# nkkk98/MyGPURaytracer

Hardware: AMD Instinct MI355X
Metric: Mrays/s (higher is better)
Workload: dtype f32; 1 GPU; cornellObj.txt 1920x1080 depth 8, AA on, material sort on, 1 spp/step (BASELINE configs[3] / C4); arith=0, clock_warmup_steps=1152, rccl_ranks=1, parallelism=1 GPU

## Files before the change

include/mi355x_pathtracer.h:

```cpp
#ifndef MI355X_PATHTRACER_H
#define MI355X_PATHTRACER_H

#include <stddef.h>
#include <stdint.h>

#ifdef __cplusplus
extern "C" {
#endif

#define PTX_ABI_VERSION 5
int ptx_abi_version(void);
size_t ptx_sizeof_options(void);
size_t ptx_sizeof_stats(void);

#define PTX_OK 0
#define PTX_ERR_INVALID 1
#define PTX_ERR_IO 2
#define PTX_ERR_HIP 3
#define PTX_ERR_NODEVICE 4
#define PTX_ERR_UNSUPPORTED 5

enum { PTX_SPHERE = 0, PTX_CUBE = 1, PTX_TRIANGLE = 2, PTX_OBJ = 3 };

typedef struct ptx_material {
// ... 217 lines not shown
                          int spp);

int ptx_kat_geom_test(ptx_tracer *t, int geom, int n, const float *rays6, float *out10);
int ptx_kat_obj_tri_test(ptx_tracer *t, int geom, int n, const float *rays6, float *out8);
int ptx_kat_jittered_hemisphere(ptx_tracer *t, int n, const float *normals3, const int32_t *seeds3, int max_iter, float *out3);
int ptx_kat_compute_intersections(ptx_tracer *t, int n, const void *paths44, void *isects32);
int ptx_kat_tile_intersect(ptx_tracer *t, int n, const void *paths44, void *isects32, int split);
int ptx_kat_shade(ptx_tracer *t, int iter, int n, const int32_t *idx, const void *isects32, void *paths44);
int ptx_kat_generate(ptx_tracer *t, int iter, void *paths44);
int ptx_kat_libm(ptx_tracer *t, int n, const float *x, float *sin_out, float *cos_out,
                 const double *pw_in, double *pow5_out, const float *powf_xy, float *powf_out);
int ptx_kat_fast_exact(ptx_tracer *t, int64_t mismatches[3]);
int ptx_debug_tile_geoms(const ptx_camera *camera, int ngeoms, const float *boxes6, int depth_of_field, int tile_rows, int tile_rank,
                         int tile_world, uint32_t *masks_out, int max_tiles);
int ptx_debug_record_masks(int nmaterials, const ptx_material *materials, int ngeoms, const int32_t *geom_type, const int32_t *geom_material,
                           int sort_by_material, uint64_t masks[2]);
int ptx_debug_cull_boxes(int n, const float *boxes6, float *centre_half8);
int ptx_debug_light_bits(int nmaterials, const ptx_material *materials, int ngeoms, const int32_t *geom_material, uint32_t *bits_out);
int ptx_debug_bounce_occupancy(ptx_tracer *t, int lds_bytes);
int ptx_debug_aux_nonzero(ptx_tracer *t, int64_t out3[3]);
int ptx_debug_set_capture(ptx_tracer *t, int bounce);
int ptx_debug_bvh_check(const float *faces15, int nfaces, const float *rays6, int nrays, int32_t *face_loop, float *t_loop,
                        int32_t *face_bvh, float *t_bvh, int64_t *stats4);
int ptx_debug_bvh_visits(int64_t out8[8]);
int ptx_debug_read_stamps(ptx_tracer *t, unsigned long long out48[48]);
int ptx_debug_read_stream(ptx_tracer *t, int *n_out, int32_t *pixel_index, int32_t *stream_idx,
                          int32_t *material, float *fields14, int cap);

#ifdef __cplusplus
}
#endif
#endif
```

mygpuraytracer_amd/csrc/pt_device.h:

```cpp
#pragma once
#include <hip/hip_runtime.h>
#include <stdint.h>

#define PT_DEV __device__ __forceinline__
#define PT_HD __host__ __device__ __forceinline__

#ifndef PT_ARITH
#define PT_ARITH 0
#endif

namespace ptd {

struct vec3 { float x, y, z; };

PT_HD vec3 V3(float x, float y, float z) { vec3 r; r.x = x; r.y = y; r.z = z; return r; }
PT_HD vec3 add(vec3 a, vec3 b) { return V3(a.x + b.x, a.y + b.y, a.z + b.z); }
PT_HD vec3 sub(vec3 a, vec3 b) { return V3(a.x - b.x, a.y - b.y, a.z - b.z); }
PT_HD vec3 mul(vec3 a, vec3 b) { return V3(a.x * b.x, a.y * b.y, a.z * b.z); }
PT_HD vec3 scale(vec3 a, float s) { return V3(a.x * s, a.y * s, a.z * s); }
PT_HD vec3 neg(vec3 a) { return V3(-a.x, -a.y, -a.z); }
PT_HD float dot(vec3 a, vec3 b) { return a.x * b.x + a.y * b.y + a.z * b.z; }
PT_HD vec3 cross(vec3 x, vec3 y) { return V3(x.y * y.z - y.y * x.z, x.z * y.x - y.z * x.x, x.x * y.y - y.x * x.y); }
#ifndef PT_FAST_EXACT
#define PT_FAST_EXACT 1
// ... 249 lines not shown
    const float *__restrict__ tri9;
    const uint8_t *__restrict__ texels;
    int32_t ngeoms, nmats;
    int32_t tri_lds;
    int32_t ntri;
    int32_t ntri_lds;
    const float *__restrict__ gtab;
    const float *__restrict__ aabb;
    uint32_t cube_bits, sphere_bits, mesh_bits;
    uint32_t light_bits;
    const BvhQuad *__restrict__ bvh_nodes;
    const float *__restrict__ bvh_tris;
    const int32_t *__restrict__ bvh_root;
    const int32_t *__restrict__ bvh_depth;
    int32_t bvh_stack;
    const BvhWide4 *__restrict__ bvh_wide;
    const int32_t *__restrict__ bvh_wroot;
    const int32_t *__restrict__ bvh_wneed;
    const float *__restrict__ fnorm;
    const float *__restrict__ cnorm;
    uint32_t bump_bits;
    int32_t mesh_chunks;
    int32_t cull;
    const float *__restrict__ ldsblob;
};

__host__ __device__ constexpr int sceneTableWords(int ntri_lds, int nmats, int ngeoms) { return (ntri_lds * 27 + nmats * 11 + ngeoms * 58 + 3) & ~3; }
PT_DEV int sceneLdsWords(const DScene &sc) { return sceneTableWords(sc.ntri_lds, sc.nmats, sc.ngeoms); }
constexpr int GTAB_WORDS = 40;

extern __shared__ __attribute__((aligned(16))) int32_t pt_lds[];

__device__ __forceinline__ void stageSceneToLds(const DScene &sc, int tid, int nthreads) {
    float *l = reinterpret_cast<float *>(pt_lds);
    if (sc.ldsblob) {
        const int n = sc.ntri_lds * 27 + sc.nmats * 11 + sc.ngeoms * 58;
        for (int k = tid; k < n; k += 4 * nthreads) {
            const int k1 = k + nthreads, k2 = k1 + nthreads, k3 = k2 + nthreads;
            const float a0 = sc.ldsblob[k], a1 = k1 < n ? sc.ldsblob[k1] : 0.f, a2 = k2 < n ? sc.ldsblob[k2] : 0.f, a3 = k3 < n ? sc.ldsblob[k3] : 0.f;
            l[k] = a0;
            if (k1 < n) l[k1] = a1;
            if (k2 < n) l[k2] = a2;
            if (k3 < n) l[k3] = a3;
        }
        return;
    }
    const int n9 = sc.ntri_lds * 9, n15 = sc.ntri_lds * 15, nm = sc.nmats * 11;
    for (int k = tid; k < n9; k += nthreads) l[k] = sc.tri9[k];
    for (int k = tid; k < n15; k += nthreads) l[n9 + k] = sc.faces[k];
    const float *m = reinterpret_cast<const float *>(sc.mats);
    for (int k = tid; k < nm; k += nthreads) l[n9 + n15 + k] = m[k];
    const int ng = sc.ngeoms * GTAB_WORDS;
// ... 162 lines not shown
    const float tiny = 1e-20f;
    const float ddx = __builtin_fabsf(d.x) < tiny ? __builtin_copysignf(tiny, d.x) : d.x;
    const float ddy = __builtin_fabsf(d.y) < tiny ? __builtin_copysignf(tiny, d.y) : d.y;
    const float ddz = __builtin_fabsf(d.z) < tiny ? __builtin_copysignf(tiny, d.z) : d.z;
    RaySlab r;
    r.ix = 1.0f / ddx; r.iy = 1.0f / ddy; r.iz = 1.0f / ddz;
    r.ox = o.x * r.ix; r.oy = o.y * r.iy; r.oz = o.z * r.iz;
    r.sx = slack * __builtin_fabsf(r.ix); r.sy = slack * __builtin_fabsf(r.iy); r.sz = slack * __builtin_fabsf(r.iz);
    return r;
}
PT_HD bool slabEntry(const BvhQuad &A, const BvhQuad &B, const RaySlab &r, float tmin, float &tn) {
    const float x0 = __builtin_fmaf(A.x, r.ix, -r.ox), x1 = __builtin_fmaf(B.x, r.ix, -r.ox);
    const float y0 = __builtin_fmaf(A.y, r.iy, -r.oy), y1 = __builtin_fmaf(B.y, r.iy, -r.oy);
    const float z0 = __builtin_fmaf(A.z, r.iz, -r.oz), z1 = __builtin_fmaf(B.z, r.iz, -r.oz);
    tn = __builtin_fmaxf(__builtin_fmaxf(__builtin_fminf(x0, x1) - r.sx, __builtin_fminf(y0, y1) - r.sy), __builtin_fminf(z0, z1) - r.sz);
    const float tf = __builtin_fminf(__builtin_fminf(__builtin_fmaxf(x0, x1) + r.sx, __builtin_fmaxf(y0, y1) + r.sy), __builtin_fmaxf(z0, z1) + r.sz);
    return !((tf < tn) || (tf < 0.0f) || (tn > tmin * 1.0001f));
}
PT_HD float bvhSlack(const BvhQuad &A, const BvhQuad &B, vec3 o) {
    const vec3 c = V3(0.5f * (A.x + B.x), 0.5f * (A.y + B.y), 0.5f * (A.z + B.z));
    const vec3 h = V3(0.5f * (B.x - A.x), 0.5f * (B.y - A.y), 0.5f * (B.z - A.z));
    const float s = 1.220703125e-4f * (length(sub(o, c)) + 4.0f * length(h));
    return s == s ? s : 3.0e38f;
}

PT_HD float bvhNearest(const BvhQuad *__restrict__ nodes, const float *__restrict__ tris, int root, vec3 o, vec3 d,
                       int &face, float &b0o, float &b1o, int *visited = nullptr) {
    const RaySlab rs = makeRaySlab(o, d, bvhSlack(nodes[2 * root], nodes[2 * root + 1], o));
    float tmin = 3.402823466e+38f;
    face = -1; b0o = 0.f; b1o = 0.f;
    int n = root;
    while (n >= 0) {
        const BvhQuad A = nodes[2 * n], B = nodes[2 * n + 1];
        float tn_;
        const bool skip = !slabEntry(A, B, rs, tmin, tn_);
        if (visited) ++*visited;
        if (skip) { n = A.w; continue; }
        const int count = (int)((uint32_t)B.w >> 28), first = B.w & 0x0fffffff;
        if (count == 0) { n = n + 1; continue; }
        for (int k = 0; k < count; k++) {
            const float *T = tris + (size_t)(first + k) * BVH_TRI;
            const vec3 v0 = V3(T[0], T[1], T[2]), p1 = V3(T[3], T[4], T[5]), p2 = V3(T[6], T[7], T[8]);
            const vec3 e1 = sub(p1, v0), e2 = sub(p2, v0);
            float b0, b1;
            if (rayTriangle(o, d, v0, e1, e2, b0, b1)) {
                const float w = 1 - b0 - b1;
// ... 869 lines not shown
```

mygpuraytracer_amd/csrc/pt_engine.hip:

```cpp
#include <hip/hip_runtime.h>
#include <stdint.h>
#include <stdio.h>
#include <string.h>
#include <string>
#include <vector>
#include <algorithm>
#include <cmath>

#include "../../include/mi355x_pathtracer.h"
#include "pt_kernels.h"
#include "pt_scene.h"
#include "pt_denoise.h"

namespace {

thread_local std::string g_last_error;
int set_error(int code, const std::string &msg) { g_last_error = msg; return code; }

#define HIPCHECK(expr)                                                                                   \
    do {                                                                                                 \
        hipError_t e_ = (expr);                                                                          \
        if (e_ != hipSuccess)                                                                            \
            return set_error(PTX_ERR_HIP, std::string(#expr) + ": " + hipGetErrorString(e_));            \
    } while (0)
// ... 266 lines not shown
    DevBuf<float> d_var;
    bool var_done = false;
    DevBuf<unsigned long long> d_stamps;
    DevBuf<float> d_part;
    DevBuf<int32_t> d_cache_totals;
    DevBuf<int32_t> d_emit_count, d_emit_pix; DevBuf<float> d_emit_rgb;
    DevBuf<int64_t> d_stats;
    uint32_t fence_slots = 0;
    int maxBounces = 0;
    bool cache_valid = false;
    int64_t iterations = 0;
    double loop_ms_total = 0.0;
    bool ktiming = false;
    std::vector<hipEvent_t> kev;
    std::vector<int> kev_kind;
    size_t kev_used = 0;
    int capture_bounce = -1;
    DevBuf<int32_t> d_cap;
    DevBuf<float> d_cap_f;
    bool cap_filled = false;
    DScene scene() const {
        DScene s; s.geoms = d_geoms; s.mats = d_mats; s.faces = d_faces; s.tri9 = d_tri9; s.texels = d_texels; s.ngeoms = ngeoms; s.nmats = nmats;
        s.gtab = d_gtab; s.aabb = d_aabb; s.cull = 0; s.cube_bits = cube_bits; s.sphere_bits = sphere_bits; s.mesh_bits = mesh_bits; s.light_bits = light_bits;
        s.bvh_nodes = d_bvh_nodes; s.bvh_tris = d_bvh_tris; s.bvh_root = d_bvh_root; s.bvh_depth = d_bvh_depth; s.bvh_wide = d_bvh_wide; s.bvh_wroot = d_bvh_wroot; s.bvh_wneed = d_bvh_wneed; s.bvh_stack = 0; s.ntri_lds = 0; s.mesh_chunks = mesh_chunks;
        s.fnorm = d_fnorm; s.cnorm = d_cnorm; s.bump_bits = bump_bits;
        s.tri_lds = 0; s.ntri = ntri;
        s.ldsblob = nullptr;
        return s;
    }
    bool cache_active() const { return opt.cache_first_bounce && !opt.antialiasing && !opt.depth_of_field; }
    const KernelSet *ks = static_cast<const KernelSet *>(ptx_arith_kernels_0());
    const LastKernelSet *ksl = static_cast<const LastKernelSet *>(ptx_arith_last_0());
};

namespace {

void carve(PathSoA &s, float *f, int32_t *i, size_t stride) {
    s.q = f; s.i = i; s.stride = (uint32_t)stride;
}

PathSoA soa_shift(PathSoA s, size_t off) {
    s.q += 4 * off; s.i += off;
    return s;
}

void fastdiv_magic(uint32_t d, uint32_t &mul, uint32_t &sh) {
    if (d <= 1) { mul = 0; sh = 255; return; }
// ... 441 lines not shown
    camera_to_device(*camera, t->cam);
    const int W = t->cam.resx, H = t->cam.resy;
    t->tm.W = W; t->tm.H = H; t->tm.tile_world = opt.tile_world; t->tm.tile_rank = opt.tile_rank;
    t->tm.tile_rows = opt.tile_world > 1 ? opt.tile_rows : H;
    fastdiv_magic((uint32_t)W, t->tm.w_mul, t->tm.w_sh);
    fastdiv_magic((uint32_t)t->tm.tile_rows, t->tm.rows_mul, t->tm.rows_sh);
    t->tm.owned = owned_pixels(W, H, t->tm.tile_rows, opt.tile_rank, opt.tile_world);
    t->maxTiles = (std::max(t->tm.owned, 1) + TILE - 1) / TILE;
    t->cap = t->maxTiles * TILE;
    t->nbins = opt.sort_by_material ? (nmaterials > 0 ? nmaterials : 1) : 1;
    {
        int per_cu = 16;
        if (const char *e = getenv("PTX_DEBUG_WG_PER_CU")) { per_cu = std::max(1, atoi(e)); t->grid_forced = true; }
        t->cus = prop.multiProcessorCount;
        t->grid = std::max(1, std::min(t->maxTiles, prop.multiProcessorCount * per_cu));
    }
    t->grid_seg = std::max(1, std::min(t->grid, t->maxTiles));
    t->nsuper = (t->grid_seg + 63) / 64;
    HostScene hs;
    SceneSwitches sw;
    sw.no_wide_bvh = getenv("PTX_DEBUG_NO_WIDE_BVH") != nullptr; sw.no_chunks = getenv("PTX_DEBUG_NO_CHUNKS") != nullptr;
    sw.no_dir_skip = getenv("PTX_DEBUG_NO_DIR_SKIP") != nullptr; sw.no_normal_codes = getenv("PTX_DEBUG_NO_NORMAL_CODES") != nullptr;
    sw.force_split = getenv("PTX_DEBUG_FORCE_SPLIT") != nullptr;
    if (const int rc = pt_prepare_scene(ngeoms, geoms, nmaterials, materials, opt, t->tm.owned, t->nbins, prop.sharedMemPerBlock, sw, hs)) return fail(rc);
    static_cast<SceneFacts &>(*t) = hs;
    {
        size_t mem_free = 0, mem_total = 0;
        if (opt.batch <= 0 && hipMemGetInfo(&mem_free, &mem_total) != hipSuccess) { mem_free = mem_total = 0; (void)hipGetLastError(); }
        const char *e = getenv("PTX_DEBUG_MEM_BUDGET_MB");
        const LaunchPlan plan = plan_launch_sets(t->tm.owned, t->nbins, t->maxTiles, opt, kmax_cap, mem_free, mem_total, e ? std::max(1LL, atoll(e)) : 0);
        if (!plan.refusal.empty()) { set_error(PTX_ERR_UNSUPPORTED, plan.refusal); return fail(PTX_ERR_UNSUPPORTED); }
        t->kmax = *kmax_used = plan.kmax;
        t->lanes = plan.lanes;
    }
    t->no_fast = getenv("PTX_DEBUG_NO_FAST") != nullptr;
    t->no_last = getenv("PTX_DEBUG_NO_LAST") != nullptr;
    t->force_fast = getenv("PTX_DEBUG_FORCE_FAST") != nullptr;
    if (const char *e = getenv("PTX_DEBUG_TOTAL_WG_PER_CU")) t->dbg_total_wg_per_cu = std::max(0, atoi(e));
    if (const char *e = getenv("PTX_DEBUG_NSETS")) t->dbg_nsets = std::max(0, atoi(e));
    if (const char *e = getenv("PTX_DEBUG_EXTRA_LDS")) t->dbg_extra_lds = std::max(0, std::min(atoi(e), 32768)) & ~15;
    if (const char *e = getenv("PTX_DEBUG_MESH_WG_PER_CU")) t->dbg_mesh_wg_per_cu = std::max(0, atoi(e));
    if (const char *e = getenv("PTX_DEBUG_SPLIT_MIN")) t->split_min_paths = std::max(1LL, atoll(e));
    if (stream) { t->stream = (hipStream_t)stream; t->own_stream = false; }
    else {
        int prio_lo = 0, prio_hi = 0;
        if (hipDeviceGetStreamPriorityRange(&prio_lo, &prio_hi) != hipSuccess) { prio_lo = prio_hi = 0; (void)hipGetLastError(); }
// ... 869 lines not shown
```

mygpuraytracer_amd/csrc/pt_kernels.h:

```cpp
#pragma once
#include <hip/hip_runtime.h>
#include <stdint.h>

#include "pt_device.h"
#include "pt_bvh.h"

using namespace ptd;

namespace {

#ifndef PT_TILE
#define PT_TILE 256
#endif
#ifndef PT_MESH_WAVES
#define PT_MESH_WAVES 5
#endif
#ifndef PT_PARK_STATE
#define PT_PARK_STATE 1
#endif
#ifndef PT_FAST_WAVES
#define PT_FAST_WAVES 8
#endif
#ifndef PT_FAST_WAVES_FIRST
#define PT_FAST_WAVES_FIRST (PT_FAST_WAVES - 1)
#endif
#ifndef PT_FAST_WAVES_SPLIT
#define PT_FAST_WAVES_SPLIT 4
#endif
#ifndef PT_FAST_WAVES_SPLIT2
#define PT_FAST_WAVES_SPLIT2 5
#endif
#ifndef PT_BOUNCE_WAVES
#define PT_BOUNCE_WAVES 4
#endif
constexpr int TILE = PT_TILE;
constexpr int WAVES = TILE / 64;
constexpr int RANK_BITS = TILE <= 256 ? 8 : 9, BIN_BITS = 32 - 2 * RANK_BITS;
static_assert(TILE <= 512 && (TILE & (TILE - 1)) == 0, "tile size: a power of two up to 512 (9-bit ranks)");
#ifndef PT_WIN
#define PT_WIN 32
#endif
constexpr int WIN = PT_WIN, WIN_WORDS = 2 * (WIN + 1) + WIN + 2;
constexpr int ldsHeadWords(int nb) { return ((2 * WAVES * nb + 4 * nb + 1 + 8 + WIN_WORDS) + 3) & ~3; }
constexpr int REC_WORDS = 17 * TILE;
#ifndef PT_REC_ROWS_FAST0
#define PT_REC_ROWS_FAST0 16
#endif
constexpr int REC_ROWS_FAST0 = PT_REC_ROWS_FAST0;
static_assert(WIN <= 64 && (WIN & (WIN - 1)) == 0, "window of runs: one wave, binary search");
__host__ __device__ constexpr size_t bounceLdsWords(int tableWords, int nb) { return (size_t)tableWords + (size_t)ldsHeadWords(nb) + REC_WORDS; }
static_assert(ldsHeadWords(1) % 4 == 0 && ldsHeadWords(2) % 4 == 0 && ldsHeadWords(3) % 4 == 0 && ldsHeadWords(7) % 4 == 0 &&
              ldsHeadWords(45) % 4 == 0 && ldsHeadWords(65535) % 4 == 0, "record buffer must start 16-byte aligned");
static_assert(sceneTableWords(1, 1, 1) % 4 == 0 && sceneTableWords(12, 7, 7) % 4 == 0 && sceneTableWords(0, 3, 5) % 4 == 0, "scene tables end 16-byte aligned");
static_assert((6 * TILE) % 2 == 0 && (8 * TILE) % 2 == 0, "tileIntersect's 64-bit keys and lists must be 8-byte aligned inside the record buffer");

#ifndef PT_QCAP
#define PT_QCAP (4 * TILE)
#endif
#ifndef PT_DIRECT_STORE
#define PT_DIRECT_STORE 1
#endif
#ifndef PT_RANK_SLICED
#define PT_RANK_SLICED 1
#endif
constexpr int QCAP = PT_QCAP;
constexpr int QUEUE_WORDS = QCAP + 4;
// ... 232 lines not shown
```

mygpuraytracer_amd/csrc/pt_kernels.hip:

```cpp
#if PT_ARITH == 1
#define ptd ptd_arith1
#elif PT_ARITH == 2
#define ptd ptd_arith2
#elif defined(PT_ARITH) && PT_ARITH != 0
#error "PT_ARITH must be 0, 1 or 2"
#endif
#include <string.h>

#include "pt_kernels.h"

namespace {

__device__ __forceinline__ int32_t stage_key(int bin, int r_all, int r_scat) { return (int32_t)((uint32_t)bin | ((uint32_t)r_all << BIN_BITS) | ((uint32_t)r_scat << (BIN_BITS + RANK_BITS))); }
__device__ __forceinline__ void fence_report(const BounceParams &p) { atomicAdd(p.fenced, 1ull); }

__device__ __forceinline__ int sum_totals(const int32_t *t, int n) {
    int s = 0;
    for (int b = 0; b < n; b++) s += t[b];
    return s;
}

constexpr int ITEMS_PER_PASS = 4;
#ifdef PT_STAMPS
#define TI_STAMP(k) do { unsigned long long t1_ = __builtin_amdgcn_s_memtime(); st_acc[k] += t1_ - st_t0; st_t0 = t1_; } while (0)
#define TI_ARGS , unsigned long long *st_acc, unsigned long long &st_t0
#define TI_PASS , st_acc, st_t0
#else
#define TI_STAMP(k) do { } while (0)
#define TI_ARGS
#define TI_PASS
#endif
template <bool DEFER, bool PARK = false, bool SUBSET = false, bool DECODE = true>
__device__ __forceinline__ void tileIntersect(const DScene &sc, bool alive, Ray ray, bool need_uv, Hit &hit, int32_t *scratch,
                                              int32_t *tcnt, int &q, int tid, int lane, int wave, unsigned long long &key_out,
                                              uint32_t &mesh_out TI_ARGS, uint32_t subset = 0xffffffffu) {
    const float *gtab = reinterpret_cast<const float *>(pt_lds) + sc.ntri_lds * 24 + sc.nmats * 11;
    float *rayb = reinterpret_cast<float *>(scratch);
    unsigned long long *best = reinterpret_cast<unsigned long long *>(scratch + 6 * TILE);
    uint16_t *list = reinterpret_cast<uint16_t *>(scratch + 8 * TILE);
    uint16_t *listM = list + ITEMS_PER_PASS * TILE;
    constexpr int CAP = ITEMS_PER_PASS * TILE;
    uint32_t cube_mask = 0, sph_mask = 0, mesh_mask = 0;
    if (alive) {
        const uint32_t m = cullMask<SUBSET>(sc, ray, subset);
        cube_mask = m & sc.cube_bits; sph_mask = m & sc.sphere_bits; mesh_mask = m & sc.mesh_bits;
    }
    mesh_out = mesh_mask;
    if (DEFER) mesh_mask = 0;
    rayb[0 * TILE + tid] = ray.o.x; rayb[1 * TILE + tid] = ray.o.y; rayb[2 * TILE + tid] = ray.o.z;
    rayb[3 * TILE + tid] = ray.d.x; rayb[4 * TILE + tid] = ray.d.y; rayb[5 * TILE + tid] = ray.d.z;
    best[tid] = KEY_NONE;
    for (;;) {
        const int cc = (int)__popc(cube_mask), cs = (int)__popc(sph_mask), cm = (int)__popc(mesh_mask);
        const int nc = cc < ITEMS_PER_PASS ? cc : ITEMS_PER_PASS;
        const int ns = cs < ITEMS_PER_PASS - nc ? cs : ITEMS_PER_PASS - nc;
        const int nm = cm < ITEMS_PER_PASS - nc - ns ? cm : ITEMS_PER_PASS - nc - ns;
        int base[3], tot[3];
        const int cnt3[3] = {nc, ns, nm};
#pragma unroll
        for (int kind = 0; kind < 3; kind++) {
            const unsigned long long b0 = __ballot(cnt3[kind] & 1), b1 = __ballot(cnt3[kind] & 2), b2 = __ballot(cnt3[kind] & 4);
            base[kind] = wavePrefix(b0, lane) + 2 * wavePrefix(b1, lane) + 4 * wavePrefix(b2, lane);
            tot[kind] = __popcll(b0) + 2 * __popcll(b1) + 4 * __popcll(b2);
// ... 7 lines not shown
            if (left) tcnt[4 * q + 3] = 1;
        }
        base[0] += __builtin_amdgcn_readfirstlane(wb0);
        base[1] += __builtin_amdgcn_readfirstlane(wb1);
        base[2] += __builtin_amdgcn_readfirstlane(wb2);
        for (int j = 0; j < nc; j++) {
            const int g = __ffs((int)cube_mask) - 1;
            cube_mask &= cube_mask - 1;
            list[base[0] + j] = (uint16_t)(tid | (g << RANK_BITS));
        }
        for (int j = 0; j < ns; j++) {
            const int g = __ffs((int)sph_mask) - 1;
            sph_mask &= sph_mask - 1;
            list[CAP - 1 - (base[1] + j)] = (uint16_t)(tid | (g << RANK_BITS));
        }
        for (int j = 0; j < nm; j++) {
            const int g = __ffs((int)mesh_mask) - 1;
            mesh_mask &= mesh_mask - 1;
            listM[base[2] + j] = (uint16_t)(tid | (g << RANK_BITS));
        }
        __syncthreads();
        const int totC = tcnt[4 * q + 0], totS = tcnt[4 * q + 1], totM = tcnt[4 * q + 2], more = tcnt[4 * q + 3];
        if (tid < 4) tcnt[4 * (q ^ 1) + tid] = 0;
        TI_STAMP(5);
#ifdef PT_STAMPS
        if (tid == 0) { st_acc[8] += totC + totS; st_acc[9] += totM; st_acc[10] += 1; }
#endif
        const int startS = (totC + 63) & ~63, startM = startS + ((totS + 63) & ~63);
        const int nch = sc.mesh_chunks > 1 ? sc.mesh_chunks : 1;
        for (int k = tid; k < startM + totM * nch; k += TILE) {
            int item = -1, chunk = -1;
            if (k < totC) item = list[k];
            else if (k >= startS && k < startS + totS) item = list[CAP - 1 - (k - startS)];
            else if (k >= startM) {
                int kk = k - startM;
                if (nch > 1) { chunk = 0; while (kk >= totM) { kk -= totM; chunk++; } }
                item = listM[kk];
            }
            if (item >= 0) {
                const int src = item & (TILE - 1), g = item >> RANK_BITS;
                Ray r;
                r.o = V3(rayb[0 * TILE + src], rayb[1 * TILE + src], rayb[2 * TILE + src]);
                r.d = V3(rayb[3 * TILE + src], rayb[4 * TILE + src], rayb[5 * TILE + src]);
                const unsigned long long key = (DEFER || k < startM) ? primKey(gtab, g, r)
                    : ((sc.tri_lds == 2 || sc.ntri_lds) ? meshKey<true>(sc, gtab, g, r, chunk) : meshKey<false>(sc, gtab, g, r, chunk));
                if (key != KEY_NONE) atomicMin(&best[src], key);
            }
        }
        __syncthreads();
        q ^= 1;
        TI_STAMP(6);
        if (!more) break;
    }
    key_out = best[tid];
    if (PARK) {
        asm volatile("" ::: "memory");
        ray.o = V3(rayb[0 * TILE + tid], rayb[1 * TILE + tid], rayb[2 * TILE + tid]);
        ray.d = V3(rayb[3 * TILE + tid], rayb[4 * TILE + tid], rayb[5 * TILE + tid]);
    }
    if (!DEFER && DECODE) decodeKey(sc, gtab, key_out, ray, need_uv, hit);
    TI_STAMP(7);
}

constexpr int32_t K1_CAND = (int32_t)0x80000000u, K1_ALIVE = 0x40000000, K1_PEND = 0x20000000;

template <bool FIRST>
__device__ __forceinline__ void classifyPath(const BounceParams &p, int iter, float *part, bool batched, const Hit &hit, vec3 color, int pix,
                                             int &bin, bool &pending) {
// ... 117 lines not shown
        p.sort = 1; p.albedo = nullptr; p.emit_count = nullptr; p.sc.cull = 1; p.sc.tri_lds = 1;
    }
    if (FAST && MODE == 0) {
        p.uses_uv = 0; p.sort = 1; p.albedo = nullptr; p.emit_count = nullptr; p.dof = 0;
        p.sc.cull = 1; p.sc.tri_lds = 2; p.sc.bump_bits = 0; p.sc.ntri_lds = p.sc.ntri; p.sc.bvh_root = nullptr;
    }
    const int tid = threadIdx.x, lane = tid & 63, wave = tid >> 6;
    const int nb = p.nbins;
    const int triWords = (MODE != 2 && p.sc.tri_lds) ? sceneLdsWords(p.sc) : 0;
    int32_t *lds = pt_lds + triWords;
    int32_t *w_all = lds, *w_scat = lds + WAVES * nb;
    int32_t *run_all = lds + 2 * WAVES * nb, *run_scat = run_all + nb;
    int32_t *tcs = run_scat + nb, *toff = tcs + nb;
    int32_t *tcnt = toff + nb + 1;
    int32_t *win = tcnt + 8;
    int tq = 0;
    int32_t *rec = lds + ldsHeadWords(nb);
    constexpr int R_PIX = (FAST && MODE == 0 ? REC_ROWS_FAST0 : 17) - 3, R_MG = R_PIX + 1, R_KEY = R_PIX + 2;
    uint32_t *qbuf = reinterpret_cast<uint32_t *>(rec + REC_WORDS);
    int32_t *qcnt = rec + REC_WORDS + QCAP, *qbase = qcnt + 1;
    if (MODE == 1 && tid == 0) *qcnt = 0;
    for (int k = tid; k < 2 * nb; k += TILE) run_all[k] = 0;
    if (tid < 8) tcnt[tid] = 0;
    __syncthreads();
    const int seg = blockIdx.y;
    const int iter = p.iter + seg * p.iter_stride;
    const PathSoA in_k = soa_offset(p.in, p.seg_in * seg), stage_k = soa_offset(p.stage, p.seg_stage * seg);
    int32_t *counts_all = p.counts_all + p.seg_counts * seg, *counts_scat = p.counts_scat + p.seg_counts * seg;
    int32_t *tile_np = counts_all + 2 * (size_t)nb * p.maxTiles;
    const bool direct = PT_DIRECT_STORE && MODE != 2 && (FAST || nb <= 64);
    int32_t *chunk_out = p.chunk + p.seg_chunk * seg;
    int32_t *super_all = p.super_all + p.seg_totals * seg, *super_scat = p.super_scat + p.seg_totals * seg;
    int32_t *totals_all = p.totals_all + p.seg_totals * seg, *totals_scat = p.totals_scat + p.seg_totals * seg;
    float *part = (FAST || p.part) ? p.part + p.seg_part * seg : nullptr;
    const bool batched = FAST || part != nullptr;
    const int32_t *in_totals = FIRST ? nullptr : p.in_totals + p.seg_in_totals * seg;
    const int32_t *in_chunk = FIRST ? nullptr : p.in_chunk + p.seg_in_chunk * seg;
    const int in_nruns = nb * p.in_gx;
    int v_tot = 0;
    if (!FIRST && nb <= 64 && lane < nb) v_tot = in_totals[nb + lane];
    const int n_in = FIRST ? p.tm.owned : nb <= 64 ? __builtin_amdgcn_readlane(waveInclusiveScan(v_tot, lane), 63) : sum_totals(in_totals + nb, nb);
    const int ntiles = (n_in + TILE - 1) / TILE;
    const int chunk = (ntiles + (int)gridDim.x - 1) / (int)gridDim.x;
    const int tile0 = min((int)blockIdx.x * chunk, ntiles), tile1 = min(tile0 + chunk, ntiles);
    auto binRanges = [&](unsigned long long mask, int &lo0, int &len0, int &lo1, int &len1) {
        int lo[2] = {0, 0}, hi[2] = {0, 0}, nr = 0, pos = 0;
// ... 794 lines not shown
    Ray r; r.o = ld3(paths[i].o); r.d = ld3(paths[i].d);
    Hit h;
    intersectScene(sc, r, h);
    HostIsect o;
    memset(&o, 0, sizeof o);
    if (h.t > 0.f) {
        o.t = h.t; o.n[0] = h.n.x; o.n[1] = h.n.y; o.n[2] = h.n.z; o.materialId = h.mat; o.uv[0] = h.u; o.uv[1] = h.v;
        o.geomId = h.geom;
    } else {
        o.t = -1.f;
    }
    out[i] = o;
}

template <bool SPLIT>
__global__ __launch_bounds__(TILE) void k_kat_tile(DScene sc, DScene scg, int n, const HostPath *paths, HostIsect *out, int uses_uv) {
    const int tid = threadIdx.x, lane = tid & 63, wave = tid >> 6;
    int32_t *lds = pt_lds + sceneLdsWords(sc);
    int32_t *tcnt = lds;
    int32_t *rec = lds + ldsHeadWords(1);
    int32_t *stack = rec + REC_WORDS;
    stageSceneToLds(sc, tid, TILE);
    if (tid < 8) tcnt[tid] = 0;
    __syncthreads();
    int tq = 0;
    const float *gtab_lds = reinterpret_cast<const float *>(pt_lds) + sc.ntri_lds * 24 + sc.nmats * 11;
    for (int base = blockIdx.x * TILE; base < n; base += gridDim.x * TILE) {
        const int i = base + tid;
        const bool alive = i < n;
        Ray ray; ray.o = ray.d = V3(0.f, 0.f, 0.f);
        if (alive) { ray.o = ld3(paths[i].o); ray.d = ld3(paths[i].d); }
        Hit h;
        h.t = -1.f; h.n = V3(0.f, 0.f, 0.f); h.u = h.v = 0.f; h.geom = 0; h.mat = 0;
        unsigned long long key = KEY_NONE;
        uint32_t mesh_cand = 0;
#ifdef PT_STAMPS
        unsigned long long st_acc[16] = {0}, st_t0 = 0;
#endif
        if (!SPLIT) {
            tileIntersect<false>(sc, alive, ray, uses_uv != 0, h, rec, tcnt, tq, tid, lane, wave, key, mesh_cand TI_PASS);
        } else {
            tileIntersect<true>(sc, alive, ray, uses_uv != 0, h, rec, tcnt, tq, tid, lane, wave, key, mesh_cand TI_PASS);
            for (uint32_t m = mesh_cand; m; m &= m - 1) {
                const unsigned long long k = meshKey(scg, scg.gtab, __ffs((int)m) - 1, ray, -1, stack + tid, TILE);
                key = k < key ? k : key;
            }
// ... 153 lines not shown
```

mygpuraytracer_amd/csrc/pt_scene.h:

```cpp
#pragma once
#include "../../include/mi355x_pathtracer.h"
#include "pt_device.h"
#include "pt_bvh.h"

namespace ptd {

struct SceneSwitches {
    bool no_wide_bvh = false;
    bool no_chunks = false;
    bool no_dir_skip = false;
    bool no_normal_codes = false;
    bool force_split = false;
};

struct SceneFacts {
    int ntri = 0, bvh_meshes = 0, bvh_nodes = 0, bvh_stack = BVH_STACK;
    int mesh_chunks = 1;
    int uses_uv = 0;
    uint32_t cube_bits = 0, sphere_bits = 0, mesh_bits = 0;
    uint32_t bump_bits = 0;
    uint32_t light_bits = 0;
    int tri_lds = 0, ntri_lds = 0, cull = 0;
    bool split_mesh = false;
    unsigned long long dir_bins = ~0ull;
    unsigned long long ntab_bins = 0ull;
};

struct HostScene : SceneFacts {
    std::vector<DGeom> geoms;
    std::vector<DMaterial> mats;
    std::vector<float> faces, tri9, gtab, fnorm, cnorm;
    std::vector<uint8_t> texels;
    std::vector<float> aabb, aabb_ch;
    std::vector<uint8_t> h_spec;
    BvhBuild bvh;
    std::vector<int32_t> roots, depths, wroots, wneeds;
    std::vector<float> ldsblob;
};

int pt_prepare_scene(int ngeoms, const ptx_geom *geoms, int nmaterials, const ptx_material *materials, const ptx_options &opt, int owned,
                     int nbins, size_t lds_limit, const SceneSwitches &sw, HostScene &out);

std::vector<float> triangle_table(const float *faces15, int nfaces);
void tile_geom_masks(const DCamera &c, int tile_rows, int tile_rank, int tile_world, int owned, int maxTiles, int ngeoms, const float *aabb8,
                     bool dof, std::vector<uint32_t> &masks);
void camera_to_device(const ptx_camera &c, DCamera &d);
int owned_pixels(int W, int H, int tile_rows, int tile_rank, int tile_world);
uint32_t light_geom_bits(int nmaterials, const DMaterial *mats, int ngeoms, const int32_t *geom_material);

}
```

mygpuraytracer_amd/csrc/pt_scene.hip:

```cpp
#include <string>

#include "pt_scene.h"
#include "pt_kernels.h"

extern "C" void ptx_internal_set_error(const char *msg);

static int set_error(int code, const std::string &msg) { ptx_internal_set_error(msg.c_str()); return code; }

namespace ptd {
void camera_to_device(const ptx_camera &c, DCamera &d) {
    d.resx = c.resolution[0]; d.resy = c.resolution[1];
    memcpy(d.position, c.position, 12); memcpy(d.lookAt, c.lookAt, 12); memcpy(d.view, c.view, 12);
    memcpy(d.up, c.up, 12); memcpy(d.right, c.right, 12); memcpy(d.fov, c.fov, 8); memcpy(d.pixelLength, c.pixelLength, 8);
}

void make_world_aabb(const DGeom &d, const std::vector<float> &faces, float out6[6]) {
    double lo[3] = {1e300, 1e300, 1e300}, hi[3] = {-1e300, -1e300, -1e300};
    bool ok = true;
    auto add = [&](double x, double y, double z) {
        for (int r = 0; r < 3; r++) {
            double v = (double)d.xf[0 * 4 + r] * x + (double)d.xf[1 * 4 + r] * y + (double)d.xf[2 * 4 + r] * z + (double)d.xf[3 * 4 + r];
            if (!(v == v) || v > 1e30 || v < -1e30) ok = false;
            lo[r] = std::min(lo[r], v); hi[r] = std::max(hi[r], v);
        }
    };
    if (d.type == G_OBJ) {
        if (d.faceCount == 0) ok = false;
        for (int j = 0; j < d.faceCount; j++)
            for (int k = 0; k < 3; k++) {
                const float *p = &faces[((size_t)d.faceStart + j) * 15 + k * 5];
                add(p[0], p[1], p[2]);
            }
    } else {
        for (int c = 0; c < 8; c++) add((c & 1) ? 0.5 : -0.5, (c & 2) ? 0.5 : -0.5, (c & 4) ? 0.5 : -0.5);
    }
    for (int r = 0; r < 3; r++) {
        if (!ok) { out6[r] = -INFINITY; out6[3 + r] = INFINITY; continue; }
        double m = 1e-3 + 1e-4 * std::max(std::fabs(lo[r]), std::fabs(hi[r]));
        out6[r] = nextafterf((float)(lo[r] - m), -INFINITY);
        out6[3 + r] = nextafterf((float)(hi[r] + m), INFINITY);
    }
}

void record_masks(int nmaterials, const DMaterial *mats, int ngeoms, const int *geom_type, const int *geom_material, bool sort,
                  unsigned long long &dir_bins, unsigned long long &ntab_bins) {
    unsigned long long need = 0, cubes = 0;
    const int nbins = sort ? nmaterials : 1;
    for (int m = 0; m < nmaterials; m++) {
        bool nd = mats[m].hasReflective > 0 || mats[m].hasRefractive > 0, on_cube = false, on_other = false;
        for (int i = 0; i < ngeoms; i++)
            if (geom_material[i] == m) { nd = nd || geom_type[i] == G_OBJ; (geom_type[i] == G_CUBE ? on_cube : on_other) = true; }
        const int b = sort ? nmaterials - 1 - m : 0;
        if (nd) need |= 1ull << b;
        if (on_cube && !on_other && sort) cubes |= 1ull << b;
    }
    auto runs = [&](unsigned long long mask) { int n = 0; for (int b = 0; b < nbins; b++) n += ((mask >> b) & 1) && !(b && ((mask >> (b - 1)) & 1)); return n; };
    while (runs(need) > 2) {
        int b = 0;
        while (!((need >> b) & 1)) b++;
        while ((need >> b) & 1) b++;
        need |= 1ull << b;
    }
    while (runs(cubes) > 2) cubes &= ~(1ull << (63 - __builtin_clzll(cubes)));
    dir_bins = need; ntab_bins = cubes;
// ... 177 lines not shown
        for (int i = 0; i < ngeoms; i++)
            if (hs.geoms[i].type == G_OBJ) hs.mesh_chunks = std::max(hs.mesh_chunks, (hs.geoms[i].faceCount + MESH_CHUNK - 1) / MESH_CHUNK);
    hs.tri_lds = (((size_t)nmaterials * 11 + (size_t)ngeoms * 58) * 4 <= 56 * 1024 && !opt.no_lds_triangles) ? 1 : 0;
    hs.ntri_lds = (hs.tri_lds && ((size_t)hs.ntri * 27 + (size_t)nmaterials * 11 + (size_t)ngeoms * 58) * 4 <= 56 * 1024) ? hs.ntri : 0;
    {
        auto need = [&]() { return sizeof(int32_t) * (bounceLdsWords(hs.tri_lds ? sceneTableWords(hs.ntri_lds, nmaterials, ngeoms) : 0, nbins) + QUEUE_WORDS); };
        if (need() > lds_limit && hs.ntri_lds) hs.ntri_lds = 0;
        if (need() > lds_limit && hs.tri_lds) hs.tri_lds = 0;
        if (need() > lds_limit)
            return set_error(PTX_ERR_UNSUPPORTED, "material sort over " + std::to_string(nbins) + " materials needs " + std::to_string(need()) +
                             " bytes of LDS per workgroup, the device offers " + std::to_string(lds_limit) + ": render with sort_by_material = 0 (same image "
                             "only if the reference is built with SORT_BY_MATERIAL 0 too)");
    }
    hs.gtab.assign(ng1 * GTAB_WORDS, 0.f); hs.aabb.assign(ng1 * 8, 0.f);
    for (int i = 0; i < ngeoms; i++) {
        const DGeom &d = hs.geoms[i];
        float *o = &hs.gtab[(size_t)i * GTAB_WORDS];
        const float *mats3[3] = {d.inv, d.xf, d.invT};
        for (int m = 0; m < 3; m++)
            for (int r = 0; r < 3; r++)
                for (int c = 0; c < 4; c++) o[m * 12 + r * 4 + c] = mats3[m][c * 4 + r];
        int32_t ints[4] = {d.type, d.materialid, d.faceStart, d.faceCount};
        memcpy(o + 36, ints, sizeof ints);
        float box[6];
        make_world_aabb(d, hs.faces, box);
        for (int k = 0; k < 3; k++) { hs.aabb[(size_t)i * 8 + k] = box[k]; hs.aabb[(size_t)i * 8 + 4 + k] = box[3 + k]; }
        if (i < 32) {
            if (d.type == G_OBJ) hs.mesh_bits |= 1u << i;
            else if (d.type == G_CUBE) hs.cube_bits |= 1u << i;
            else if (d.type == G_SPHERE) hs.sphere_bits |= 1u << i;
        }
    }
    hs.aabb_ch.assign(hs.aabb.size(), 0.f);
    for (int i = 0; i < ngeoms; i++) world_box_centre_half(&hs.aabb[(size_t)i * 8], &hs.aabb_ch[(size_t)i * 8]);
    hs.cull = (hs.tri_lds && ngeoms >= 1 && ngeoms <= 32 && !opt.no_cull) ? 1 : 0;
    hs.fnorm.assign((size_t)std::max(hs.ntri, 1) * 3, 0.f); hs.cnorm.assign(ng1 * 18, 0.f);
    for (int i = 0; i < ngeoms; i++) {
        const DGeom &d = hs.geoms[i];
        if (d.type == G_OBJ) {
            if (d.tex[3].ch && i < 32) hs.bump_bits |= 1u << i;
            for (int j = 0; j < d.faceCount; j++) {
                const float *tri = &hs.faces[((size_t)d.faceStart + j) * 15];
                const vec3 e1 = sub(ld3(tri + 5), ld3(tri)), e2 = sub(ld3(tri + 10), ld3(tri));
                const vec3 objN = normalize(cross(e1, e2));
                const vec3 n = normalize(multiplyMV(d.invT, objN, 0.f));
                float *o = &hs.fnorm[((size_t)d.faceStart + j) * 3];
                o[0] = n.x; o[1] = n.y; o[2] = n.z;
            }
        } else if (d.type == G_CUBE) {
            const float *invT = &hs.gtab[(size_t)i * GTAB_WORDS + 24];
            for (int side = 0; side < 6; side++) {
                const int axis = side >> 1;
                const float sgn = (side & 1) ? 1.f : -1.f;
                const vec3 e = V3(axis == 0 ? sgn : 0.f, axis == 1 ? sgn : 0.f, axis == 2 ? sgn : 0.f);
                const vec3 n = normalize(mulRows(invT, e, 0.0f));
                float *o = &hs.cnorm[(size_t)i * 18 + side * 3];
                o[0] = n.x; o[1] = n.y; o[2] = n.z;
            }
// ... 75 lines not shown
            if (i % 64 == 63 || i == nrays - 1) { sum_group_max += group_max; group_max = 0; groups++; }
            if (wstack[(size_t)std::max(wneed, 1)] != 0x7fffffff) mismatches += 1000000;
            if (f3 != f1 || memcmp(&t3, &t_bvh[i], 4) != 0 || (f1 >= 0 && (memcmp(&e0, &b0, 4) != 0 || memcmp(&e1, &b1, 4) != 0))) mismatches++;
            {
                WideWalk w;
                wideStart(w, bb.nodes[2 * (size_t)root], bb.nodes[2 * (size_t)root + 1], wroot, o, d);
                while (w.n != WIDE_DONE) {
                    if (w.n >= 0) wideNodeStep(w, bb.wide.data(), wstack.data(), 1);
                    else wideLeafStep<true>(w, bb.tris.data(), wstack.data(), 1);
                }
                if (wstack[(size_t)std::max(wneed, 1)] != 0x7fffffff) mismatches += 1000000;
                if (w.face != f1 || memcmp(&w.tmin, &t_bvh[i], 4) != 0 || (f1 >= 0 && (memcmp(&w.b0, &b0, 4) != 0 || memcmp(&w.b1, &b1, 4) != 0))) mismatches++;
            }
        }
        face_loop[i] = f0; face_bvh[i] = f1;
        visited += vis;
    }
    if (stats4) { stats4[0] = (int64_t)(bb.nodes.size() / 2); stats4[1] = (int64_t)(bb.tris.size() / BVH_TRI); stats4[2] = visited; stats4[3] = mismatches; }
    g_bvh_visits[0] = visited; g_bvh_visits[1] = visited_ordered; g_bvh_visits[2] = visited_wide / 4; g_bvh_visits[3] = wneed;
    g_bvh_visits[4] = sum_group_max; g_bvh_visits[5] = groups; g_bvh_visits[6] = tris_wide;
    return PTX_OK;
}

int ptx_debug_record_masks(int nmaterials, const ptx_material *materials, int ngeoms, const int32_t *geom_type, const int32_t *geom_material,
                           int sort_by_material, uint64_t masks[2]) {
    if (nmaterials < 1 || nmaterials > 64 || !materials || ngeoms < 0 || (ngeoms && (!geom_type || !geom_material)) || !masks)
    { set_error(PTX_ERR_INVALID, "ptx_debug_record_masks: bad argument"); return -1; }
    unsigned long long d = 0, n = 0;
    record_masks(nmaterials, reinterpret_cast<const DMaterial *>(materials), ngeoms, geom_type, geom_material, sort_by_material != 0, d, n);
    masks[0] = d; masks[1] = n;
    return 0;
}

int ptx_debug_light_bits(int nmaterials, const ptx_material *materials, int ngeoms, const int32_t *geom_material, uint32_t *bits_out) {
    if (nmaterials < 0 || (nmaterials && !materials) || ngeoms < 0 || (ngeoms && !geom_material) || !bits_out)
    { set_error(PTX_ERR_INVALID, "ptx_debug_light_bits: bad argument"); return -1; }
    *bits_out = light_geom_bits(nmaterials, reinterpret_cast<const DMaterial *>(materials), ngeoms, geom_material);
    return 0;
}

int ptx_debug_cull_boxes(int n, const float *boxes6, float *centre_half8) {
    if (n < 0 || (n && (!boxes6 || !centre_half8))) { set_error(PTX_ERR_INVALID, "ptx_debug_cull_boxes: bad argument"); return -1; }
    for (int g = 0; g < n; g++) {
        const float lohi[8] = {boxes6[g * 6], boxes6[g * 6 + 1], boxes6[g * 6 + 2], 0.f, boxes6[g * 6 + 3], boxes6[g * 6 + 4], boxes6[g * 6 + 5], 0.f};
        world_box_centre_half(lohi, centre_half8 + (size_t)g * 8);
    }
// ... 31 lines not shown
```

Before: 42860 Mrays/s.

## Cull mesh candidates with an object-space box test before triangle loops

Adds a conservative object-space bounding box per mesh, stored in spare words of the geometry table, and tests each ray-mesh pair against it in the tile intersect kernel. Surviving pairs are compacted with a ballot and atomic counter into a survivor list, and only those run the full triangle (chunked) intersection. This removes full mesh loops for rays that miss the mesh box, at the cost of an extra transform, a slab test, an atomic, and a block barrier per pass. It is active only when meshes are not using the BVH path.

```diff
diff --git a/include/mi355x_pathtracer.h b/include/mi355x_pathtracer.h
--- a/include/mi355x_pathtracer.h
+++ b/include/mi355x_pathtracer.h
@@ -263,6 +263,8 @@
 int ptx_debug_set_capture(ptx_tracer *t, int bounce);
 int ptx_debug_bvh_check(const float *faces15, int nfaces, const float *rays6, int nrays, int32_t *face_loop, float *t_loop,
                         int32_t *face_bvh, float *t_bvh, int64_t *stats4);
+int ptx_debug_mesh_box_check(const float *faces15, int nfaces, const float *inverse16, const float *rays6, int nrays, uint8_t *reached,
+                             int32_t *accepted, float *box10);
 int ptx_debug_bvh_visits(int64_t out8[8]);
 int ptx_debug_read_stamps(ptx_tracer *t, unsigned long long out48[48]);
 int ptx_debug_read_stream(ptx_tracer *t, int *n_out, int32_t *pixel_index, int32_t *stream_idx,
diff --git a/mygpuraytracer_amd/csrc/pt_device.h b/mygpuraytracer_amd/csrc/pt_device.h
--- a/mygpuraytracer_amd/csrc/pt_device.h
+++ b/mygpuraytracer_amd/csrc/pt_device.h
@@ -295,12 +295,17 @@
     uint32_t bump_bits;
     int32_t mesh_chunks;
     int32_t cull;
+    int32_t mesh_box;
     const float *__restrict__ ldsblob;
 };
 
 __host__ __device__ constexpr int sceneTableWords(int ntri_lds, int nmats, int ngeoms) { return (ntri_lds * 27 + nmats * 11 + ngeoms * 58 + 3) & ~3; }
 PT_DEV int sceneLdsWords(const DScene &sc) { return sceneTableWords(sc.ntri_lds, sc.nmats, sc.ngeoms); }
 constexpr int GTAB_WORDS = 40;
+constexpr int MESH_BOX_AT = 12, MESH_BOX_WORDS = 10;
+static_assert(MESH_BOX_AT + MESH_BOX_WORDS <= 24, "the box lies inside the forward transform's words");
+static_assert(sizeof(DScene) == 200 && __builtin_offsetof(DScene, ldsblob) == 192 && __builtin_offsetof(DScene, mesh_box) == 188,
+              "DScene::mesh_box fills padding: the fields k_mesh, k_finish and the ranking pass read stay where they were");
 
 extern __shared__ __attribute__((aligned(16))) int32_t pt_lds[];
 
@@ -509,6 +514,15 @@
     const vec3 h = V3(0.5f * (B.x - A.x), 0.5f * (B.y - A.y), 0.5f * (B.z - A.z));
     const float s = 1.220703125e-4f * (length(sub(o, c)) + 4.0f * length(h));
     return s == s ? s : 3.0e38f;
+}
+PT_HD bool meshBoxReached(const float *box10, vec3 o, vec3 d) {
+    BvhQuad A, B;
+    A.x = box10[0]; A.y = box10[1]; A.z = box10[2]; A.w = 0;
+    B.x = box10[3]; B.y = box10[4]; B.z = box10[5]; B.w = 0;
+    const float l1 = (__builtin_fabsf(o.x - box10[6]) + __builtin_fabsf(o.y - box10[7])) + (__builtin_fabsf(o.z - box10[8]) + box10[9]);
+    const float s = 1.220703125e-4f * l1;
+    float tn;
+    return slabEntry(A, B, makeRaySlab(o, d, s == s ? s : 3.0e38f), 3.402823466e+38f, tn);
 }
 
 PT_HD float bvhNearest(const BvhQuad *__restrict__ nodes, const float *__restrict__ tris, int root, vec3 o, vec3 d,
diff --git a/mygpuraytracer_amd/csrc/pt_engine.hip b/mygpuraytracer_amd/csrc/pt_engine.hip
--- a/mygpuraytracer_amd/csrc/pt_engine.hip
+++ b/mygpuraytracer_amd/csrc/pt_engine.hip
@@ -312,7 +312,7 @@
     DScene scene() const {
         DScene s; s.geoms = d_geoms; s.mats = d_mats; s.faces = d_faces; s.tri9 = d_tri9; s.texels = d_texels; s.ngeoms = ngeoms; s.nmats = nmats;
         s.gtab = d_gtab; s.aabb = d_aabb; s.cull = 0; s.cube_bits = cube_bits; s.sphere_bits = sphere_bits; s.mesh_bits = mesh_bits; s.light_bits = light_bits;
-        s.bvh_nodes = d_bvh_nodes; s.bvh_tris = d_bvh_tris; s.bvh_root = d_bvh_root; s.bvh_depth = d_bvh_depth; s.bvh_wide = d_bvh_wide; s.bvh_wroot = d_bvh_wroot; s.bvh_wneed = d_bvh_wneed; s.bvh_stack = 0; s.ntri_lds = 0; s.mesh_chunks = mesh_chunks;
+        s.bvh_nodes = d_bvh_nodes; s.bvh_tris = d_bvh_tris; s.bvh_root = d_bvh_root; s.bvh_depth = d_bvh_depth; s.bvh_wide = d_bvh_wide; s.bvh_wroot = d_bvh_wroot; s.bvh_wneed = d_bvh_wneed; s.bvh_stack = 0; s.ntri_lds = 0; s.mesh_chunks = mesh_chunks; s.mesh_box = mesh_box;
         s.fnorm = d_fnorm; s.cnorm = d_cnorm; s.bump_bits = bump_bits;
         s.tri_lds = 0; s.ntri = ntri;
         s.ldsblob = nullptr;
@@ -800,6 +800,7 @@
     sw.no_wide_bvh = getenv("PTX_DEBUG_NO_WIDE_BVH") != nullptr; sw.no_chunks = getenv("PTX_DEBUG_NO_CHUNKS") != nullptr;
     sw.no_dir_skip = getenv("PTX_DEBUG_NO_DIR_SKIP") != nullptr; sw.no_normal_codes = getenv("PTX_DEBUG_NO_NORMAL_CODES") != nullptr;
     sw.force_split = getenv("PTX_DEBUG_FORCE_SPLIT") != nullptr;
+    sw.no_mesh_box = getenv("PTX_DEBUG_NO_MESH_BOX") != nullptr;
     if (const int rc = pt_prepare_scene(ngeoms, geoms, nmaterials, materials, opt, t->tm.owned, t->nbins, prop.sharedMemPerBlock, sw, hs)) return fail(rc);
     static_cast<SceneFacts &>(*t) = hs;
     {
diff --git a/mygpuraytracer_amd/csrc/pt_kernels.h b/mygpuraytracer_amd/csrc/pt_kernels.h
--- a/mygpuraytracer_amd/csrc/pt_kernels.h
+++ b/mygpuraytracer_amd/csrc/pt_kernels.h
@@ -42,6 +42,8 @@
 #endif
 constexpr int WIN = PT_WIN, WIN_WORDS = 2 * (WIN + 1) + WIN + 2;
 constexpr int ldsHeadWords(int nb) { return ((2 * WAVES * nb + 4 * nb + 1 + 8 + WIN_WORDS) + 3) & ~3; }
+constexpr int SURV_AT = 8 + WIN_WORDS;
+static_assert((2 * WAVES + 4) % 4 == 0 && (1 + 8 + WIN_WORDS) % 4 == 1, "the survivor counters fit the head's padding");
 constexpr int REC_WORDS = 17 * TILE;
 #ifndef PT_REC_ROWS_FAST0
 #define PT_REC_ROWS_FAST0 16
diff --git a/mygpuraytracer_amd/csrc/pt_kernels.hip b/mygpuraytracer_amd/csrc/pt_kernels.hip
--- a/mygpuraytracer_amd/csrc/pt_kernels.hip
+++ b/mygpuraytracer_amd/csrc/pt_kernels.hip
@@ -39,6 +39,7 @@
     unsigned long long *best = reinterpret_cast<unsigned long long *>(scratch + 6 * TILE);
     uint16_t *list = reinterpret_cast<uint16_t *>(scratch + 8 * TILE);
     uint16_t *listM = list + ITEMS_PER_PASS * TILE;
+    int32_t *tsurv = tcnt + SURV_AT;
     constexpr int CAP = ITEMS_PER_PASS * TILE;
     uint32_t cube_mask = 0, sph_mask = 0, mesh_mask = 0;
     if (alive) {
@@ -92,28 +93,88 @@
         __syncthreads();
         const int totC = tcnt[4 * q + 0], totS = tcnt[4 * q + 1], totM = tcnt[4 * q + 2], more = tcnt[4 * q + 3];
         if (tid < 4) tcnt[4 * (q ^ 1) + tid] = 0;
+        if (!DEFER && tid == 4) tsurv[q ^ 1] = 0;
         TI_STAMP(5);
 #ifdef PT_STAMPS
         if (tid == 0) { st_acc[8] += totC + totS; st_acc[9] += totM; st_acc[10] += 1; }
 #endif
         const int startS = (totC + 63) & ~63, startM = startS + ((totS + 63) & ~63);
         const int nch = sc.mesh_chunks > 1 ? sc.mesh_chunks : 1;
-        for (int k = tid; k < startM + totM * nch; k += TILE) {
-            int item = -1, chunk = -1;
-            if (k < totC) item = list[k];
-            else if (k >= startS && k < startS + totS) item = list[CAP - 1 - (k - startS)];
-            else if (k >= startM) {
-                int kk = k - startM;
-                if (nch > 1) { chunk = 0; while (kk >= totM) { kk -= totM; chunk++; } }
-                item = listM[kk];
-            }
-            if (item >= 0) {
+        if (DEFER) {
+            for (int k = tid; k < startM + totM * nch; k += TILE) {
+                int item = -1, chunk = -1;
+                if (k < totC) item = list[k];
+                else if (k >= startS && k < startS + totS) item = list[CAP - 1 - (k - startS)];
+                else if (k >= startM) {
+                    int kk = k - startM;
+                    if (nch > 1) { chunk = 0; while (kk >= totM) { kk -= totM; chunk++; } }
+                    item = listM[kk];
+                }
+                (void)chunk;
+                if (item >= 0) {
+                    const int src = item & (TILE - 1), g = item >> RANK_BITS;
+                    Ray r;
+                    r.o = V3(rayb[0 * TILE + src], rayb[1 * TILE + src], rayb[2 * TILE + src]);
+                    r.d = V3(rayb[3 * TILE + src], rayb[4 * TILE + src], rayb[5 * TILE + src]);
+                    const unsigned long long key = primKey(gtab, g, r);
+                    if (key != KEY_NONE) atomicMin(&best[src], key);
+                }
+            }
+        } else {
+            const bool boxed = sc.mesh_box != 0;
+            uint16_t *surv = list + totC;
+            const int end1 = startM + (boxed ? totM : 0);
+            for (int k = tid; k < end1; k += TILE) {
+                if (k >= startM) {
+                    const int item = listM[k - startM];
+                    const int src = item & (TILE - 1), g = item >> RANK_BITS;
+                    const float *G = gtab + g * GTAB_WORDS;
+                    float inv[12];
+#pragma unroll
+                    for (int j = 0; j < 12; j++) inv[j] = G[j];
+                    Ray oq;
+                    oq.o = mulRows(inv, V3(rayb[0 * TILE + src], rayb[1 * TILE + src], rayb[2 * TILE + src]), 1.0f);
+                    oq.d = normalize(mulRows(inv, V3(rayb[3 * TILE + src], rayb[4 * TILE + src], rayb[5 * TILE + src]), 0.0f));
+                    const bool keep = meshBoxReached(G + MESH_BOX_AT, oq.o, oq.d);
+                    const unsigned long long kb = __ballot(keep);
+                    int wb = 0;
+                    if (lane == 0 && kb) wb = atomicAdd(&tsurv[q], __popcll(kb));
+                    const int slot = __builtin_amdgcn_readfirstlane(wb) + wavePrefix(kb, lane);
+                    if (keep && (unsigned)slot < (unsigned)totM) surv[slot] = (uint16_t)item;
+                    continue;
+                }
+                int item = -1;
+                if (k < totC) item = list[k];
+                else if (k >= startS && k < startS + totS) item = list[CAP - 1 - (k - startS)];
+                if (item >= 0) {
+                    const int src = item & (TILE - 1), g = item >> RANK_BITS;
+                    Ray r;
+                    r.o = V3(rayb[0 * TILE + src], rayb[1 * TILE + src], rayb[2 * TILE + src]);
+                    r.d = V3(rayb[3 * TILE + src], rayb[4 * TILE + src], rayb[5 * TILE + src]);
+                    const unsigned long long key = primKey(gtab, g, r);
+                    if (key != KEY_NONE) atomicMin(&best[src], key);
+                }
+            }
+            int nsurv = totM;
+            const uint16_t *pairs = listM;
+            if (boxed && totM > 0) {
+                __syncthreads();
+                nsurv = tsurv[q];
+                nsurv = nsurv < totM ? nsurv : totM;
+                pairs = surv;
+            }
+#ifdef PT_STAMPS
+            if (tid == 0) st_acc[15] += nsurv;
+#endif
+            for (int k = (tid - ((end1 + 63) & ~63)) & (TILE - 1); k < nsurv * nch; k += TILE) {
+                int kk = k, chunk = -1;
+                if (nch > 1) { chunk = 0; while (kk >= nsurv) { kk -= nsurv; chunk++; } }
+                const int item = pairs[kk];
                 const int src = item & (TILE - 1), g = item >> RANK_BITS;
                 Ray r;
                 r.o = V3(rayb[0 * TILE + src], rayb[1 * TILE + src], rayb[2 * TILE + src]);
                 r.d = V3(rayb[3 * TILE + src], rayb[4 * TILE + src], rayb[5 * TILE + src]);
-                const unsigned long long key = (DEFER || k < startM) ? primKey(gtab, g, r)
-                    : ((sc.tri_lds == 2 || sc.ntri_lds) ? meshKey<true>(sc, gtab, g, r, chunk) : meshKey<false>(sc, gtab, g, r, chunk));
+                const unsigned long long key = (sc.tri_lds == 2 || sc.ntri_lds) ? meshKey<true>(sc, gtab, g, r, chunk) : meshKey<false>(sc, gtab, g, r, chunk);
                 if (key != KEY_NONE) atomicMin(&best[src], key);
             }
         }
@@ -277,6 +338,7 @@
     if (MODE == 1 && tid == 0) *qcnt = 0;
     for (int k = tid; k < 2 * nb; k += TILE) run_all[k] = 0;
     if (tid < 8) tcnt[tid] = 0;
+    if (MODE == 0 && tid < 2) tcnt[SURV_AT + tid] = 0;
     __syncthreads();
     const int seg = blockIdx.y;
     const int iter = p.iter + seg * p.iter_stride;
@@ -1117,6 +1179,7 @@
     int32_t *stack = rec + REC_WORDS;
     stageSceneToLds(sc, tid, TILE);
     if (tid < 8) tcnt[tid] = 0;
+    if (!SPLIT && tid < 2) tcnt[SURV_AT + tid] = 0;
     __syncthreads();
     int tq = 0;
     const float *gtab_lds = reinterpret_cast<const float *>(pt_lds) + sc.ntri_lds * 24 + sc.nmats * 11;
diff --git a/mygpuraytracer_amd/csrc/pt_scene.h b/mygpuraytracer_amd/csrc/pt_scene.h
--- a/mygpuraytracer_amd/csrc/pt_scene.h
+++ b/mygpuraytracer_amd/csrc/pt_scene.h
@@ -11,11 +11,13 @@
     bool no_dir_skip = false;
     bool no_normal_codes = false;
     bool force_split = false;
+    bool no_mesh_box = false;
 };
 
 struct SceneFacts {
     int ntri = 0, bvh_meshes = 0, bvh_nodes = 0, bvh_stack = BVH_STACK;
     int mesh_chunks = 1;
+    int mesh_box = 0;
     int uses_uv = 0;
     uint32_t cube_bits = 0, sphere_bits = 0, mesh_bits = 0;
     uint32_t bump_bits = 0;
@@ -47,5 +49,6 @@
 void camera_to_device(const ptx_camera &c, DCamera &d);
 int owned_pixels(int W, int H, int tile_rows, int tile_rank, int tile_world);
 uint32_t light_geom_bits(int nmaterials, const DMaterial *mats, int ngeoms, const int32_t *geom_material);
+void mesh_object_box(const DGeom &d, const std::vector<float> &faces, float out[MESH_BOX_WORDS]);
 
 }
diff --git a/mygpuraytracer_amd/csrc/pt_scene.hip b/mygpuraytracer_amd/csrc/pt_scene.hip
--- a/mygpuraytracer_amd/csrc/pt_scene.hip
+++ b/mygpuraytracer_amd/csrc/pt_scene.hip
@@ -40,6 +40,37 @@
         out6[r] = nextafterf((float)(lo[r] - m), -INFINITY);
         out6[3 + r] = nextafterf((float)(hi[r] + m), INFINITY);
     }
+}
+
+void mesh_object_box(const DGeom &d, const std::vector<float> &faces, float out[MESH_BOX_WORDS]) {
+    double lo[3] = {1e300, 1e300, 1e300}, hi[3] = {-1e300, -1e300, -1e300};
+    bool ok = d.faceCount > 0 && ((size_t)d.faceStart + (size_t)d.faceCount) * 15 <= faces.size();
+    for (int j = 0; ok && j < d.faceCount; j++)
+        for (int k = 0; k < 3; k++) {
+            const float *p = &faces[((size_t)d.faceStart + j) * 15 + k * 5];
+            for (int r = 0; r < 3; r++) {
+                const double v = p[r];
+                if (!(v == v) || v > 1e30 || v < -1e30) ok = false;
+                lo[r] = std::min(lo[r], v); hi[r] = std::max(hi[r], v);
+            }
+        }
+    if (!ok) {
+        for (int r = 0; r < 3; r++) { out[r] = -INFINITY; out[3 + r] = INFINITY; out[6 + r] = 0.f; }
+        out[9] = INFINITY;
+        return;
+    }
+    double diag = 0.0;
+    for (int r = 0; r < 3; r++) diag += (hi[r] - lo[r]) * (hi[r] - lo[r]);
+    diag = std::sqrt(diag);
+    const double m = 2e-3 * diag + 1e-5 * diag + 1e-30;
+    double hd = 0.0;
+    for (int r = 0; r < 3; r++) {
+        out[r] = nextafterf((float)(lo[r] - m), -INFINITY);
+        out[3 + r] = nextafterf((float)(hi[r] + m), INFINITY);
+        out[6 + r] = (float)(0.5 * ((double)out[r] + (double)out[3 + r]));
+        hd += 0.25 * ((double)out[3 + r] - (double)out[r]) * ((double)out[3 + r] - (double)out[r]);
+    }
+    out[9] = nextafterf((float)(4.0 * std::sqrt(hd) * 1.001), INFINITY);
 }
 
 void record_masks(int nmaterials, const DMaterial *mats, int ngeoms, const int *geom_type, const int *geom_material, bool sort,
@@ -263,6 +294,7 @@
                 for (int c = 0; c < 4; c++) o[m * 12 + r * 4 + c] = mats3[m][c * 4 + r];
         int32_t ints[4] = {d.type, d.materialid, d.faceStart, d.faceCount};
         memcpy(o + 36, ints, sizeof ints);
+        if (d.type == G_OBJ) mesh_object_box(d, hs.faces, o + MESH_BOX_AT);
         float box[6];
         make_world_aabb(d, hs.faces, box);
         for (int k = 0; k < 3; k++) { hs.aabb[(size_t)i * 8 + k] = box[k]; hs.aabb[(size_t)i * 8 + 4 + k] = box[3 + k]; }
@@ -275,6 +307,7 @@
     hs.aabb_ch.assign(hs.aabb.size(), 0.f);
     for (int i = 0; i < ngeoms; i++) world_box_centre_half(&hs.aabb[(size_t)i * 8], &hs.aabb_ch[(size_t)i * 8]);
     hs.cull = (hs.tri_lds && ngeoms >= 1 && ngeoms <= 32 && !opt.no_cull) ? 1 : 0;
+    hs.mesh_box = (!hs.bvh_meshes && hs.mesh_bits != 0u && !sw.no_mesh_box) ? 1 : 0;
     hs.fnorm.assign((size_t)std::max(hs.ntri, 1) * 3, 0.f); hs.cnorm.assign(ng1 * 18, 0.f);
     for (int i = 0; i < ngeoms; i++) {
         const DGeom &d = hs.geoms[i];
@@ -396,6 +429,36 @@
     return PTX_OK;
 }
 
+int ptx_debug_mesh_box_check(const float *faces15, int nfaces, const float *inverse16, const float *rays6, int nrays, uint8_t *reached,
+                             int32_t *accepted, float *box10) {
+    if (nfaces < 0 || (nfaces && !faces15) || !inverse16 || nrays < 0 || (nrays && (!rays6 || !reached || !accepted)))
+        return set_error(PTX_ERR_INVALID, "ptx_debug_mesh_box_check: bad argument");
+    std::vector<float> faces;
+    if (nfaces) faces.assign(faces15, faces15 + (size_t)nfaces * 15);
+    const std::vector<float> tri9 = triangle_table(faces.data(), nfaces);
+    DGeom d;
+    memset(&d, 0, sizeof d);
+    d.type = G_OBJ; d.faceStart = 0; d.faceCount = nfaces;
+    float box[MESH_BOX_WORDS], inv[12];
+    mesh_object_box(d, faces, box);
+    if (box10) memcpy(box10, box, sizeof box);
+    for (int r = 0; r < 3; r++)
+        for (int c = 0; c < 4; c++) inv[r * 4 + c] = inverse16[c * 4 + r];
+    for (int i = 0; i < nrays; i++) {
+        const vec3 o = mulRows(inv, V3(rays6[i * 6 + 0], rays6[i * 6 + 1], rays6[i * 6 + 2]), 1.0f);
+        const vec3 dir = normalize(mulRows(inv, V3(rays6[i * 6 + 3], rays6[i * 6 + 4], rays6[i * 6 + 5]), 0.0f));
+        reached[i] = meshBoxReached(box, o, dir) ? 1 : 0;
+        int n = 0;
+        for (int j = 0; j < nfaces; j++) {
+            const float *t9 = &tri9[(size_t)j * 9];
+            float b0, b1;
+            if (rayTriangle(o, dir, V3(t9[0], t9[1], t9[2]), V3(t9[3], t9[4], t9[5]), V3(t9[6], t9[7], t9[8]), b0, b1)) n++;
+        }
+        accepted[i] = n;
+    }
+    return PTX_OK;
+}
+
 int ptx_debug_record_masks(int nmaterials, const ptx_material *materials, int ngeoms, const int32_t *geom_type, const int32_t *geom_material,
                            int sort_by_material, uint64_t masks[2]) {
     if (nmaterials < 1 || nmaterials > 64 || !materials || ngeoms < 0 || (ngeoms && (!geom_type || !geom_material)) || !masks)
```

New measurement: 41620 Mrays/s. -2.9%, worse.
